# alibaba/easydist

Measured on AMD Instinct MI355X. Metric: gpt2_train_samples_per_sec, higher is better.
Workload: dtype bf16; 1 GPU; model=gpt2-small, global_batch=64, seq_len=1024, parallelism=auto(dp1)

## Files before the change

### easydist_amd/ops/csrc/attn_kernels.hip

```cpp
#include "common.h"
#include "attn_block_map.h"
#include <torch/extension.h>
#include <ATen/cuda/CUDAContext.h>
#include <climits>

using f32x4 = __attribute__((ext_vector_type(4))) float;
using bf16x8v = __attribute__((ext_vector_type(8))) __bf16;

#define QB 64
#define KB 64

DEVINL int lsw(int e) { return e ^ (((e >> 7) & 15) << 3); }


DEVINL void swp_pack(const f32x4* sacc, int nj, unsigned pk[][2]) {
  for (int j = 0; j < nj; ++j)
    #pragma unroll
    for (int t2 = 0; t2 < 2; ++t2)
      asm("v_cvt_pk_bf16_f32 %0, %1, %2"
          : "=v"(pk[j][t2])
          : "v"(sacc[j][2 * t2]), "v"(sacc[j][2 * t2 + 1]));
}

DEVINL bf16x8v swp_butterfly(const unsigned pk[][2], int ks, int fg) {
  unsigned o0 = pk[2 * ks][0], o1 = pk[2 * ks][1];
  unsigned p0 = pk[2 * ks + 1][0], p1 = pk[2 * ks + 1][1];
  const bool g_odd = (fg & 1), g_hi = (fg >= 2);
  unsigned r16a = __shfl_xor((int)(g_odd ? o0 : p0), 16, WAVE);
  unsigned r16b = __shfl_xor((int)(g_odd ? o1 : p1), 16, WAVE);
  unsigned r32a = __shfl_xor((int)(g_hi ? o0 : p0), 32, WAVE);
  unsigned r32b = __shfl_xor((int)(g_hi ? o1 : p1), 32, WAVE);
  unsigned r48a = __shfl_xor((int)(fg == 2 ? o0 : p0), 48, WAVE);
  unsigned r48b = __shfl_xor((int)(fg == 2 ? o1 : p1), 48, WAVE);
  union { unsigned u[4]; bf16x8v v; } cv;
  if (fg == 0) {
    cv.u[0] = o0;  cv.u[1] = o1;  cv.u[2] = r16a; cv.u[3] = r16b;
  } else if (fg == 1) {
    cv.u[0] = r48a; cv.u[1] = r48b; cv.u[2] = r32a; cv.u[3] = r32b;
  } else if (fg == 2) {
    cv.u[0] = r32a; cv.u[1] = r32b; cv.u[2] = r48a; cv.u[3] = r48b;
  } else {
    cv.u[0] = r16a; cv.u[1] = r16b; cv.u[2] = p0;  cv.u[3] = p1;
  }
  return cv.v;
}

template <int D>
__global__ void
__launch_bounds__(512, (D == 64 ? 4 : 1))
flash_fwd_kernel(const bf16* __restrict__ Q, const bf16* __restrict__ K,
                 const bf16* __restrict__ V, bf16* __restrict__ O,
                 float* __restrict__ LSE, int B, int H, int S, bool causal,
                 float scale,
                 long qsb, long qsh, long qss, long ksb, long ksh, long kss,
                 long vsb, long vsh, long vss, int map_mode) {
  constexpr int QBLK = 2 * QB;
  const AttnBlock wgm = attn_block_map(blockIdx.x, (S + QBLK - 1) / QBLK,
                                       B * H, causal, map_mode);
  const int qb0 = wgm.blk * QBLK;
  const int bh = wgm.bh;
  const int b_ = bh / H, h_ = bh % H;
  const bf16* q = Q + b_ * qsb + h_ * qsh;
  const bf16* k = K + b_ * ksb + h_ * ksh;
  const bf16* v = V + b_ * vsb + h_ * vsh;
  bf16* o = O + (long)bh * S * D;
  float* lse = LSE + (long)bh * S;

  const int lane = threadIdx.x % WAVE;
  const int wave = threadIdx.x / WAVE;

  extern __shared__ __attribute__((aligned(16))) char smem[];
  constexpr int TILE_K = KB * D;
  constexpr int TILE_VT = KB * D;
  bf16* smem_b = reinterpret_cast<bf16*>(smem);
  constexpr int NTHR = 8 * WAVE;

  const int fr = lane & 15;
  const int fg = lane >> 4;

  const int qr0 = qb0 + wave * 16;
  const int qrow = qr0 + fr;

  const float qscale = scale * 1.44269504088896340736f;
  bf16x8v qf[D / 32];
  #pragma unroll
  for (int ks = 0; ks < D / 32; ++ks) {
    if (qrow < S) {
      bf16x8v raw = *reinterpret_cast<const bf16x8v*>(
          &q[(long)qrow * qss + ks * 32 + fg * 8]);
      #pragma unroll
      for (int u = 0; u < 8; ++u)
        qf[ks][u] = (__bf16)(bf2f((bf16)raw[u]) * qscale);
    } else {
      #pragma unroll
      for (int u = 0; u < 8; ++u) qf[ks][u] = (__bf16)0.f;
    }
  }

  float m_run = -1e30f, l_run = 0.f;
  f32x4 o_acc[D / 16];
  #pragma unroll
  for (int j = 0; j < D / 16; ++j) o_acc[j] = {0.f, 0.f, 0.f, 0.f};

  const int kv_end = causal ? min(S, qb0 + QBLK) : S;
  const int n_tiles = (kv_end + KB - 1) / KB;
  constexpr int PF = TILE_K / (NTHR * 8);
  bf16x8 kreg[PF], vreg[PF];

  auto load_tile = [&](int t) {
    #pragma unroll
    for (int pi = 0; pi < PF; ++pi) {
      const int e = threadIdx.x * 8 + pi * (NTHR * 8);
      const int row = t * KB + e / D, col = e % D;
      kreg[pi] = *reinterpret_cast<const bf16x8*>(&k[(long)row * kss + col]);
      vreg[pi] = *reinterpret_cast<const bf16x8*>(&v[(long)row * vss + col]);
    }
  };
  auto store_tile = [&](int t) {
    bf16* kb = smem_b + (t & 1) * (TILE_K + TILE_VT);
    bf16* vb = kb + TILE_K;
    #pragma unroll
    for (int pi = 0; pi < PF; ++pi) {
      const int e = threadIdx.x * 8 + pi * (NTHR * 8);
      *reinterpret_cast<bf16x8*>(&kb[lsw(e)]) = kreg[pi];
      const int row = e / D, col = e % D;
      #pragma unroll
      for (int i = 0; i < 8; ++i)
        vb[lsw((col + i) * KB + row)] = vreg[pi].v[i];
    }
  };

  load_tile(0);
  store_tile(0);
  __syncthreads();

  for (int t = 0; t < n_tiles; ++t) {
    const int kv0 = t * KB;
    const bf16* k_lds = smem_b + (t & 1) * (TILE_K + TILE_VT);
    const bf16* vt_lds = k_lds + TILE_K;
    if (t + 1 < n_tiles)
      load_tile(t + 1);

    const bool wave_active = !(causal && kv0 > qr0 + 15);
    if (wave_active) {
      f32x4 s_acc[KB / 16];
      __builtin_amdgcn_s_setprio(1);
      #pragma unroll
      for (int j = 0; j < KB / 16; ++j) {
        s_acc[j] = {0.f, 0.f, 0.f, 0.f};
        #pragma unroll
        for (int ks = 0; ks < D / 32; ++ks) {
          bf16x8v kf = *reinterpret_cast<const bf16x8v*>(
              &k_lds[lsw((j * 16 + fr) * D + ks * 32 + fg * 8)]);
          s_acc[j] = __builtin_amdgcn_mfma_f32_16x16x32_bf16(
              kf, qf[ks], s_acc[j], 0, 0, 0);
        }
      }
      __builtin_amdgcn_s_setprio(0);
      const bool need_mask = (causal && kv0 + KB - 1 > qrow)
                             || (kv0 + KB > S);
      float mx = -1e30f;
      if (need_mask) {
        #pragma unroll
        for (int j = 0; j < KB / 16; ++j)
          #pragma unroll
          for (int r = 0; r < 4; ++r) {
            int kcol = kv0 + j * 16 + 4 * fg + r;
            float sv = s_acc[j][r];
            if ((causal && kcol > qrow) || kcol >= S) sv = -1e30f;
            s_acc[j][r] = sv;
            mx = fmaxf(mx, sv);
          }
      } else {
        #pragma unroll
        for (int j = 0; j < KB / 16; ++j)
          #pragma unroll
          for (int r = 0; r < 4; ++r) mx = fmaxf(mx, s_acc[j][r]);
      }
      mx = fmaxf(mx, __shfl_xor(mx, 16, WAVE));
      mx = fmaxf(mx, __shfl_xor(mx, 32, WAVE));
      float m_new = fmaxf(m_run, mx);
      float psum = 0.f;
      #pragma unroll
      for (int j = 0; j < KB / 16; ++j)
        #pragma unroll
        for (int r = 0; r < 4; ++r) {
          float pp = __builtin_amdgcn_exp2f(s_acc[j][r] - m_new);
          s_acc[j][r] = pp;
          psum += pp;
        }
      psum += __shfl_xor(psum, 16, WAVE);
      psum += __shfl_xor(psum, 32, WAVE);
      float alpha = __builtin_amdgcn_exp2f(m_run - m_new);
      l_run = l_run * alpha + psum;
      m_run = m_new;
      #pragma unroll
      for (int r = 0; r < 4; ++r) {
        float ar = __shfl(alpha, 4 * fg + r, WAVE);
        #pragma unroll
        for (int j = 0; j < D / 16; ++j) o_acc[j][r] *= ar;
      }
      unsigned pk[KB / 16][2];
      swp_pack(s_acc, KB / 16, pk);
      __builtin_amdgcn_s_setprio(1);
      #pragma unroll
      for (int ks = 0; ks < KB / 32; ++ks) {
        bf16x8v pv = swp_butterfly(pk, ks, fg);
        #pragma unroll
        for (int j = 0; j < D / 16; ++j) {
          bf16x8v vf = *reinterpret_cast<const bf16x8v*>(
              &vt_lds[lsw((j * 16 + fr) * KB + ks * 32 + fg * 8)]);
          o_acc[j] = __builtin_amdgcn_mfma_f32_16x16x32_bf16(
              pv, vf, o_acc[j], 0, 0, 0);
        }
      }
      __builtin_amdgcn_s_setprio(0);
    }

    if (t + 1 < n_tiles)
      store_tile(t + 1);
    __syncthreads();
  }

  float invl = 1.f / l_run;
  #pragma unroll
  for (int r = 0; r < 4; ++r) {
    int orow = qr0 + 4 * fg + r;
    if (orow >= S) continue;
    float ir = __shfl(invl, 4 * fg + r, WAVE);
    #pragma unroll
    for (int j = 0; j < D / 16; ++j)
      o[(long)orow * D + j * 16 + fr] = f2bf(o_acc[j][r] * ir);
  }
  if (fg == 0 && qrow < S)
    lse[qrow] = 0.69314718055994530942f * (m_run + __log2f(l_run));
}

static inline at::Tensor ed_attn_arg(const at::Tensor& t) {
  return t.stride(3) == 1 ? t : t.contiguous();
}

static inline int ed_attn_map_mode() {
  const char* e = getenv("EASYDIST_ATTN_MAP");
  return (e && atoi(e) == 0) ? ATTN_MAP_LEGACY : ATTN_MAP_BALANCED;
}

static inline dim3 ed_attn_grid(long nblk, long nbh, const char* who) {
  TORCH_CHECK(nblk * nbh <= (long)INT_MAX, who,
              ": workgroup count ", nblk * nbh, " does not fit in an int");
  return dim3((unsigned)(nblk * nbh));
}

std::tuple<at::Tensor, at::Tensor> flash_attn_fwd(const at::Tensor& q_,
                                                  const at::Tensor& k_,
                                                  const at::Tensor& v_,
                                                  bool causal) {
  auto q = ed_attn_arg(q_), k = ed_attn_arg(k_), v = ed_attn_arg(v_);
  TORCH_CHECK(q.dtype() == at::kBFloat16 && q.dim() == 4);
  TORCH_CHECK(q.sizes() == k.sizes() && q.sizes() == v.sizes(),
              "flash_attn_fwd: q/k/v shapes must match");
  const int B = q.size(0), H = q.size(1), S = q.size(2), D = q.size(3);
  TORCH_CHECK(D == 64 || D == 128, "flash_attn_fwd: D in {64,128}");
  TORCH_CHECK(S % QB == 0, "flash_attn_fwd: S multiple of 64");
  auto out = at::empty({B, H, S, D}, q.options());
  auto lse = at::empty({B, H, S}, q.options().dtype(at::kFloat));
  auto stream = at::cuda::getCurrentCUDAStream();
  dim3 grid = ed_attn_grid((S + 2 * QB - 1) / (2 * QB), (long)B * H,
                           "flash_attn_fwd"), block(512);
  const int map_mode = ed_attn_map_mode();
  size_t lds = (2 * ((size_t)KB * D + (size_t)KB * D) + 8 * 16 * KB) * 2;
  float scale = 1.f / sqrtf((float)D);
  auto kern = (D == 64) ? flash_fwd_kernel<64> : flash_fwd_kernel<128>;
  hipLaunchKernelGGL(kern, grid, block, lds, stream,
      (const bf16*)q.data_ptr(), (const bf16*)k.data_ptr(),
      (const bf16*)v.data_ptr(), (bf16*)out.data_ptr(),
      lse.data_ptr<float>(), B, H, S, causal, scale,
      q.stride(0), q.stride(1), q.stride(2),
      k.stride(0), k.stride(1), k.stride(2),
      v.stride(0), v.stride(1), v.stride(2), map_mode);
  return {out, lse};
}


template <int D>
__global__ void __launch_bounds__(512)
flash_bwd_dq_kernel(const bf16* __restrict__ dO, const bf16* __restrict__ Q,
                    const bf16* __restrict__ K, const bf16* __restrict__ V,
                    const float* __restrict__ LSE,
                    const float* __restrict__ DELTA, bf16* __restrict__ DQ,
                    int B, int H, int S, bool causal, float scale,
                    long dsb, long dsh, long dss, long qsb, long qsh,
                    long qss, long ksb, long ksh, long kss, long vsb,
                    long vsh, long vss, long osb, long osh, long oss,
                    int map_mode) {
  const AttnBlock wgm = attn_block_map(blockIdx.x, S / (2 * QB), B * H,
                                       causal, map_mode);
  const int qb0 = wgm.blk * (2 * QB);
  const int bh = wgm.bh;
  const int b_ = bh / H, h_ = bh % H;
  const bf16* dO_ = dO + b_ * dsb + h_ * dsh;
  const bf16* q = Q + b_ * qsb + h_ * qsh;
  const bf16* k = K + b_ * ksb + h_ * ksh;
  const bf16* v = V + b_ * vsb + h_ * vsh;
  bf16* dq = DQ + b_ * osb + h_ * osh;
  const float* lse = LSE + (long)bh * S;
  const float* delta = DELTA + (long)bh * S;

  const int lane = threadIdx.x % WAVE;
  const int wave = threadIdx.x / WAVE;
  const int qr0 = qb0 + wave * 16;
  const int fr = lane & 15;
  const int fg = lane >> 4;

  extern __shared__ __attribute__((aligned(16))) char smem[];
  constexpr int DQBUF = 3 * KB * D;
  bf16* k_lds = reinterpret_cast<bf16*>(smem);
  bf16* v_lds = k_lds + KB * D;
  bf16* kt_lds = v_lds + KB * D;

  bf16x8v qf[D / 32], dof[D / 32];
  #pragma unroll
  for (int ks = 0; ks < D / 32; ++ks) {
    qf[ks] = *reinterpret_cast<const bf16x8v*>(
        &q[(long)(qr0 + fr) * qss + ks * 32 + fg * 8]);
    dof[ks] = *reinterpret_cast<const bf16x8v*>(
        &dO_[(long)(qr0 + fr) * dss + ks * 32 + fg * 8]);
  }
  const int qrow = qr0 + fr;
  const float lse_r = lse[qrow];
  const float dlt_r = delta[qrow];

  f32x4 dq_acc[D / 16];
  #pragma unroll
  for (int j = 0; j < D / 16; ++j) dq_acc[j] = {0.f, 0.f, 0.f, 0.f};

  const int kv_end = causal ? min(S, qb0 + 2 * QB) : S;
  constexpr int NV = KB * D / (512 * 8);
  bf16x8 kreg[NV], vreg[NV];
  auto kv_load = [&](int t0) {
    #pragma unroll
    for (int pi = 0; pi < NV; ++pi) {
      const int e = threadIdx.x * 8 + pi * 4096;
      const long row = t0 + e / D;
      const int col = e % D;
      kreg[pi] = *reinterpret_cast<const bf16x8*>(&k[row * kss + col]);
      vreg[pi] = *reinterpret_cast<const bf16x8*>(&v[row * vss + col]);
    }
  };
  auto kv_store = [&](int buf) {
    #pragma unroll
    for (int pi = 0; pi < NV; ++pi) {
      const int e = threadIdx.x * 8 + pi * 4096;
      *reinterpret_cast<bf16x8*>(&k_lds[buf * DQBUF + lsw(e)]) = kreg[pi];
      *reinterpret_cast<bf16x8*>(&v_lds[buf * DQBUF + lsw(e)]) = vreg[pi];
      const int row = e / D, col = e % D;
      #pragma unroll
      for (int i = 0; i < 8; ++i)
        kt_lds[buf * DQBUF + lsw((col + i) * KB + row)] = kreg[pi].v[i];
    }
  };
  kv_load(0);
  kv_store(0);
  __syncthreads();
  const int n_kt = (kv_end + KB - 1) / KB;
  for (int tt = 0; tt < n_kt; ++tt) {
    const int kv0 = tt * KB;
    const int bofs = (tt & 1) * DQBUF;
    if (tt + 1 < n_kt) kv_load(kv0 + KB);
    if (causal && kv0 > qr0 + 15) {
      if (tt + 1 < n_kt) kv_store((tt + 1) & 1);
      __syncthreads();
      continue;
    }

    f32x4 s_acc[KB / 16], dp_acc[KB / 16];
    #pragma unroll
    for (int j = 0; j < KB / 16; ++j) {
      s_acc[j] = {0.f, 0.f, 0.f, 0.f};
      dp_acc[j] = {0.f, 0.f, 0.f, 0.f};
      #pragma unroll
      for (int ks = 0; ks < D / 32; ++ks) {
        bf16x8v kf = *reinterpret_cast<const bf16x8v*>(
            &k_lds[bofs + lsw((j * 16 + fr) * D + ks * 32 + fg * 8)]);
        bf16x8v vf = *reinterpret_cast<const bf16x8v*>(
            &v_lds[bofs + lsw((j * 16 + fr) * D + ks * 32 + fg * 8)]);
        s_acc[j] = __builtin_amdgcn_mfma_f32_16x16x32_bf16(
            kf, qf[ks], s_acc[j], 0, 0, 0);
        dp_acc[j] = __builtin_amdgcn_mfma_f32_16x16x32_bf16(
            vf, dof[ks], dp_acc[j], 0, 0, 0);
      }
    }
    const bool need_mask = (causal && kv0 + KB - 1 > qrow)
                           || (kv0 + KB > S);
    #pragma unroll
    for (int j = 0; j < KB / 16; ++j)
      #pragma unroll
      for (int r = 0; r < 4; ++r) {
        float p = 0.f;
        int kcol = kv0 + j * 16 + 4 * fg + r;
        if (!need_mask || (!(causal && kcol > qrow) && kcol < S))
          p = __expf(s_acc[j][r] * scale - lse_r);
        s_acc[j][r] = p * (dp_acc[j][r] - dlt_r) * scale;
      }
    bf16x8v dsf[KB / 32];
    unsigned pk[KB / 16][2];
    swp_pack(s_acc, KB / 16, pk);
    #pragma unroll
    for (int ks = 0; ks < KB / 32; ++ks)
      dsf[ks] = swp_butterfly(pk, ks, fg);
    #pragma unroll
    for (int j = 0; j < D / 16; ++j) {
      #pragma unroll
      for (int ks = 0; ks < KB / 32; ++ks) {
        bf16x8v kcol = *reinterpret_cast<const bf16x8v*>(
            &kt_lds[bofs + lsw((j * 16 + fr) * KB + ks * 32 + fg * 8)]);
        dq_acc[j] = __builtin_amdgcn_mfma_f32_16x16x32_bf16(dsf[ks], kcol,
                                                            dq_acc[j], 0, 0,
                                                            0);
      }
    }
    if (tt + 1 < n_kt) kv_store((tt + 1) & 1);
    __syncthreads();
  }
  #pragma unroll
  for (int r = 0; r < 4; ++r) {
    int orow = qr0 + 4 * fg + r;
    if (orow >= S) continue;
    #pragma unroll
    for (int j = 0; j < D / 16; ++j)
      dq[(long)orow * oss + j * 16 + fr] = f2bf(dq_acc[j][r]);
  }
}

template <int D, int SW = 0>
__global__ void __launch_bounds__(512)
flash_bwd_dkv_kernel(const bf16* __restrict__ dO, const bf16* __restrict__ Q,
                     const bf16* __restrict__ K, const bf16* __restrict__ V,
                     const float* __restrict__ LSE,
                     const float* __restrict__ DELTA, bf16* __restrict__ DK,
                     bf16* __restrict__ DV, int B, int H, int S, bool causal,
                     float scale,
                     long dsb, long dsh, long dss, long qsb, long qsh,
                     long qss, long ksb, long ksh, long kss, long vsb,
                     long vsh, long vss, long osb, long osh, long oss,
                     int map_mode) {
  const AttnBlock wgm = attn_block_map(blockIdx.x, S / (2 * KB), B * H,
                                       false, map_mode);
  const int kb0 = wgm.blk * (2 * KB);
  const int bh = wgm.bh;
  const int b_ = bh / H, h_ = bh % H;
  const bf16* dO_ = dO + b_ * dsb + h_ * dsh;
  const bf16* q = Q + b_ * qsb + h_ * qsh;
  const bf16* k = K + b_ * ksb + h_ * ksh;
  const bf16* v = V + b_ * vsb + h_ * vsh;
  bf16* dk = DK + b_ * osb + h_ * osh;
  bf16* dv = DV + b_ * osb + h_ * osh;
  const float* lse = LSE + (long)bh * S;
  const float* delta = DELTA + (long)bh * S;

  const int lane = threadIdx.x % WAVE;
  const int wave = threadIdx.x / WAVE;
  const int kr0 = kb0 + wave * 16;
  const int fr = lane & 15;
  const int fg = lane >> 4;

  extern __shared__ __attribute__((aligned(16))) char smem[];
  constexpr int KVBUF = 4 * QB * D;
  bf16* q_lds = reinterpret_cast<bf16*>(smem);
  bf16* do_lds = q_lds + QB * D;
  bf16* qt_lds = do_lds + QB * D;
  bf16* dot_lds = qt_lds + QB * D;
  bf16* s_lds = reinterpret_cast<bf16*>(smem) + 2 * KVBUF + wave * 16 * QB;

  bf16x8v kf[D / 32], vf[D / 32];
  #pragma unroll
  for (int ks = 0; ks < D / 32; ++ks) {
    kf[ks] = *reinterpret_cast<const bf16x8v*>(
        &k[(long)(kr0 + fr) * kss + ks * 32 + fg * 8]);
    vf[ks] = *reinterpret_cast<const bf16x8v*>(
        &v[(long)(kr0 + fr) * vss + ks * 32 + fg * 8]);
  }

  f32x4 dk_acc[D / 16], dv_acc[D / 16];
  #pragma unroll
  for (int j = 0; j < D / 16; ++j) {
    dk_acc[j] = {0.f, 0.f, 0.f, 0.f};
    dv_acc[j] = {0.f, 0.f, 0.f, 0.f};
  }

  const int q_start = causal ? kb0 : 0;
  constexpr int NV = QB * D / (512 * 8);
  bf16x8 qreg[NV], dreg[NV];
  auto q_load = [&](int t0) {
    #pragma unroll
    for (int pi = 0; pi < NV; ++pi) {
      const int e = threadIdx.x * 8 + pi * 4096;
      const long row = t0 + e / D;
      const int col = e % D;
      qreg[pi] = *reinterpret_cast<const bf16x8*>(&q[row * qss + col]);
      dreg[pi] = *reinterpret_cast<const bf16x8*>(&dO_[row * dss + col]);
    }
  };
  auto q_store = [&](int buf) {
    #pragma unroll
    for (int pi = 0; pi < NV; ++pi) {
      const int e = threadIdx.x * 8 + pi * 4096;
      *reinterpret_cast<bf16x8*>(&q_lds[buf * KVBUF + lsw(e)]) = qreg[pi];
      *reinterpret_cast<bf16x8*>(&do_lds[buf * KVBUF + lsw(e)]) = dreg[pi];
      const int row = e / D, col = e % D;
      #pragma unroll
      for (int i = 0; i < 8; ++i) {
        qt_lds[buf * KVBUF + lsw((col + i) * QB + row)] = qreg[pi].v[i];
        dot_lds[buf * KVBUF + lsw((col + i) * QB + row)] = dreg[pi].v[i];
      }
    }
  };
  q_load(q_start);
  q_store(0);
  __syncthreads();
  const int n_qt = (S - q_start + QB - 1) / QB;
  for (int tt = 0; tt < n_qt; ++tt) {
    const int q0 = q_start + tt * QB;
    const int bofs = (tt & 1) * KVBUF;
    if (tt + 1 < n_qt) q_load(q0 + QB);
    if (causal && q0 + QB - 1 < kr0) {
      if (tt + 1 < n_qt) q_store((tt + 1) & 1);
      __syncthreads();
      continue;
    }

    f32x4 st_acc[QB / 16], dpt_acc[QB / 16];
    #pragma unroll
    for (int j = 0; j < QB / 16; ++j) {
      st_acc[j] = {0.f, 0.f, 0.f, 0.f};
      dpt_acc[j] = {0.f, 0.f, 0.f, 0.f};
      #pragma unroll
      for (int ks = 0; ks < D / 32; ++ks) {
        bf16x8v qfb = *reinterpret_cast<const bf16x8v*>(
            &q_lds[bofs + lsw((j * 16 + fr) * D + ks * 32 + fg * 8)]);
        bf16x8v dob = *reinterpret_cast<const bf16x8v*>(
            &do_lds[bofs + lsw((j * 16 + fr) * D + ks * 32 + fg * 8)]);
        if (SW) {
          st_acc[j] = __builtin_amdgcn_mfma_f32_16x16x32_bf16(
              qfb, kf[ks], st_acc[j], 0, 0, 0);
          dpt_acc[j] = __builtin_amdgcn_mfma_f32_16x16x32_bf16(
              dob, vf[ks], dpt_acc[j], 0, 0, 0);
        } else {
          st_acc[j] = __builtin_amdgcn_mfma_f32_16x16x32_bf16(
              kf[ks], qfb, st_acc[j], 0, 0, 0);
          dpt_acc[j] = __builtin_amdgcn_mfma_f32_16x16x32_bf16(
              vf[ks], dob, dpt_acc[j], 0, 0, 0);
        }
      }
    }
    bf16x8v ptf[QB / 32];
    const bool need_mask = (causal && kr0 + 15 > q0) || (q0 + QB > S);
    if (SW) {
      const int krow = kr0 + fr;
      #pragma unroll
      for (int j = 0; j < QB / 16; ++j) {
        f32x4 l4 = *reinterpret_cast<const f32x4*>(
            &lse[q0 + j * 16 + 4 * fg]);
        #pragma unroll
        for (int r = 0; r < 4; ++r) {
          int qcol = q0 + j * 16 + 4 * fg + r;
          float p = 0.f;
          if (!need_mask || (!(causal && krow > qcol) && qcol < S))
            p = __expf(st_acc[j][r] * scale - l4[r]);
          st_acc[j][r] = p;
        }
      }
      unsigned pk[QB / 16][2];
      swp_pack(st_acc, QB / 16, pk);
      #pragma unroll
      for (int ks = 0; ks < QB / 32; ++ks)
        ptf[ks] = swp_butterfly(pk, ks, fg);
    } else {
    if (need_mask) {
      #pragma unroll
      for (int j = 0; j < QB / 16; ++j) {
        int qcol = q0 + j * 16 + fr;
        float l = lse[qcol];
        #pragma unroll
        for (int r = 0; r < 4; ++r) {
          int krow = kr0 + 4 * fg + r;
          float p = 0.f;
          if (!(causal && krow > qcol) && qcol < S)
            p = __expf(st_acc[j][r] * scale - l);
          st_acc[j][r] = p;
          s_lds[lsw((4 * fg + r) * QB + j * 16 + fr)] = f2bf(p);
        }
      }
    } else {
      #pragma unroll
      for (int j = 0; j < QB / 16; ++j) {
        float l = lse[q0 + j * 16 + fr];
        #pragma unroll
        for (int r = 0; r < 4; ++r) {
          float p = __expf(st_acc[j][r] * scale - l);
          st_acc[j][r] = p;
          s_lds[lsw((4 * fg + r) * QB + j * 16 + fr)] = f2bf(p);
        }
      }
    }
    lds_fence();
    #pragma unroll
    for (int ks = 0; ks < QB / 32; ++ks)
      ptf[ks] = *reinterpret_cast<const bf16x8v*>(
          &s_lds[lsw(fr * QB + ks * 32 + fg * 8)]);
    }
    #pragma unroll
    for (int j = 0; j < D / 16; ++j) {
      #pragma unroll
      for (int ks = 0; ks < QB / 32; ++ks) {
        bf16x8v docol = *reinterpret_cast<const bf16x8v*>(
            &dot_lds[bofs + lsw((j * 16 + fr) * QB + ks * 32 + fg * 8)]);
        dv_acc[j] = __builtin_amdgcn_mfma_f32_16x16x32_bf16(ptf[ks], docol,
                                                            dv_acc[j], 0, 0,
                                                            0);
      }
    }
    bf16x8v dstf[QB / 32];
    if (SW) {
      #pragma unroll
      for (int j = 0; j < QB / 16; ++j) {
        f32x4 d4 = *reinterpret_cast<const f32x4*>(
            &delta[q0 + j * 16 + 4 * fg]);
        #pragma unroll
        for (int r = 0; r < 4; ++r) {
          float ds = st_acc[j][r] * (dpt_acc[j][r] - d4[r]) * scale;
          st_acc[j][r] = ds;
        }
      }
      unsigned pk2[QB / 16][2];
      swp_pack(st_acc, QB / 16, pk2);
      #pragma unroll
      for (int ks = 0; ks < QB / 32; ++ks)
        dstf[ks] = swp_butterfly(pk2, ks, fg);
    } else {
    lds_fence();
    #pragma unroll
    for (int j = 0; j < QB / 16; ++j) {
      int qcol = q0 + j * 16 + fr;
      float dlt = delta[qcol];
      #pragma unroll
      for (int r = 0; r < 4; ++r) {
        float ds = st_acc[j][r] * (dpt_acc[j][r] - dlt) * scale;
        s_lds[lsw((4 * fg + r) * QB + j * 16 + fr)] = f2bf(ds);
      }
    }
    lds_fence();
    #pragma unroll
    for (int ks = 0; ks < QB / 32; ++ks)
      dstf[ks] = *reinterpret_cast<const bf16x8v*>(
          &s_lds[lsw(fr * QB + ks * 32 + fg * 8)]);
    }
    #pragma unroll
    for (int j = 0; j < D / 16; ++j) {
      #pragma unroll
      for (int ks = 0; ks < QB / 32; ++ks) {
        bf16x8v qcolf = *reinterpret_cast<const bf16x8v*>(
            &qt_lds[bofs + lsw((j * 16 + fr) * QB + ks * 32 + fg * 8)]);
        dk_acc[j] = __builtin_amdgcn_mfma_f32_16x16x32_bf16(dstf[ks], qcolf,
                                                            dk_acc[j], 0, 0,
                                                            0);
      }
    }
    if (tt + 1 < n_qt) q_store((tt + 1) & 1);
    __syncthreads();
  }
  #pragma unroll
  for (int r = 0; r < 4; ++r) {
    int krow = kr0 + 4 * fg + r;
    if (krow >= S) continue;
    #pragma unroll
    for (int j = 0; j < D / 16; ++j) {
      dk[(long)krow * oss + j * 16 + fr] = f2bf(dk_acc[j][r]);
      dv[(long)krow * oss + j * 16 + fr] = f2bf(dv_acc[j][r]);
    }
  }
}

template <int D>
__global__ void __launch_bounds__(256)
attn_delta_kernel(const bf16* __restrict__ dO, const bf16* __restrict__ O,
                  float* __restrict__ delta, long rows, int H, int S,
                  long dsb, long dsh, long dss) {
  constexpr int LPR = D / 8;
  const int lane = threadIdx.x % WAVE;
  const int wave = threadIdx.x / WAVE;
  constexpr int RPW = WAVE / LPR;
  long row = (long)blockIdx.x * (4 * RPW) + wave * RPW + lane / LPR;
  if (row >= rows) return;
  const int c0 = (lane % LPR) * 8;
  const long b_ = row / ((long)H * S), hs = row % ((long)H * S);
  const long h_ = hs / S, s_ = hs % S;
  const bf16x8 d8 = *reinterpret_cast<const bf16x8*>(
      &dO[b_ * dsb + h_ * dsh + s_ * dss + c0]);
  const bf16x8 o8 = *reinterpret_cast<const bf16x8*>(&O[row * D + c0]);
  float acc = 0.f;
  #pragma unroll
  for (int i = 0; i < 8; ++i) acc += bf2f(d8.v[i]) * bf2f(o8.v[i]);
  #pragma unroll
  for (int off = LPR / 2; off > 0; off >>= 1)
    acc += __shfl_down(acc, off, WAVE);
  if (lane % LPR == 0) delta[row] = acc;
}

static void
flash_attn_bwd_launch(const at::Tensor& grad_, const at::Tensor& q_,
                      const at::Tensor& k_, const at::Tensor& v_,
                      const at::Tensor& out, const at::Tensor& lse,
                      bool causal, bf16* dq_p, bf16* dk_p, bf16* dv_p,
                      long osb, long osh, long oss) {
  auto grad = ed_attn_arg(grad_);
  auto q = ed_attn_arg(q_), k = ed_attn_arg(k_), v = ed_attn_arg(v_);
  TORCH_CHECK(q.dtype() == at::kBFloat16 && q.dim() == 4);
  TORCH_CHECK(q.sizes() == k.sizes() && q.sizes() == v.sizes());
  TORCH_CHECK(out.is_contiguous(), "flash_attn_bwd: out must be contiguous");
  const int B = q.size(0), H = q.size(1), S = q.size(2), D = q.size(3);
  TORCH_CHECK(D == 64 || D == 128, "flash_attn_bwd: D in {64,128}");
  TORCH_CHECK(S % (2 * QB) == 0, "flash_attn_bwd: S multiple of 128");
  auto delta = at::empty({B, H, S}, q.options().dtype(at::kFloat));
  {
    long rows = (long)B * H * S;
    int rpw = (D == 64) ? 8 : 4;
    long nblk = (rows + 4 * rpw - 1) / (4 * rpw);
    auto stream0 = at::cuda::getCurrentCUDAStream();
    auto dkern = (D == 64) ? attn_delta_kernel<64> : attn_delta_kernel<128>;
    hipLaunchKernelGGL(dkern, dim3(nblk), dim3(256), 0,
        stream0, (const bf16*)grad.data_ptr(), (const bf16*)out.data_ptr(),
        delta.data_ptr<float>(), rows, H, S,
        grad.stride(0), grad.stride(1), grad.stride(2));
  }
  auto stream = at::cuda::getCurrentCUDAStream();
  dim3 grid = ed_attn_grid(S / (2 * QB), (long)B * H, "flash_attn_bwd"),
       block(512);
  const int map_mode = ed_attn_map_mode();
  size_t lds = (2 * (3 * (size_t)KB * D) + 8 * 16 * KB) * 2;
  size_t lds_kv = (2 * (4 * (size_t)QB * D) + 8 * 16 * QB) * 2;
  float scale = 1.f / sqrtf((float)D);
  auto qkern = (D == 64) ? flash_bwd_dq_kernel<64> : flash_bwd_dq_kernel<128>;
  static int swkv = []() {
    const char* e = getenv("EASYDIST_DKV_SWAP");
    return e ? atoi(e) : 0;
  }();
  auto kkern = (D == 64)
      ? (swkv ? flash_bwd_dkv_kernel<64, 1> : flash_bwd_dkv_kernel<64>)
      : (swkv ? flash_bwd_dkv_kernel<128, 1> : flash_bwd_dkv_kernel<128>);
  hipLaunchKernelGGL(qkern, grid, block, lds, stream,
      (const bf16*)grad.data_ptr(), (const bf16*)q.data_ptr(),
      (const bf16*)k.data_ptr(), (const bf16*)v.data_ptr(),
      lse.data_ptr<float>(), delta.data_ptr<float>(),
      dq_p, B, H, S, causal, scale,
      grad.stride(0), grad.stride(1), grad.stride(2),
      q.stride(0), q.stride(1), q.stride(2),
      k.stride(0), k.stride(1), k.stride(2),
      v.stride(0), v.stride(1), v.stride(2), osb, osh, oss, map_mode);
  hipLaunchKernelGGL(kkern, grid, block, lds_kv, stream,
      (const bf16*)grad.data_ptr(), (const bf16*)q.data_ptr(),
      (const bf16*)k.data_ptr(), (const bf16*)v.data_ptr(),
      lse.data_ptr<float>(), delta.data_ptr<float>(),
      dk_p, dv_p, B, H, S, causal, scale,
      grad.stride(0), grad.stride(1), grad.stride(2),
      q.stride(0), q.stride(1), q.stride(2),
      k.stride(0), k.stride(1), k.stride(2),
      v.stride(0), v.stride(1), v.stride(2), osb, osh, oss, map_mode);
}

std::tuple<at::Tensor, at::Tensor, at::Tensor>
flash_attn_bwd(const at::Tensor& grad_, const at::Tensor& q_,
               const at::Tensor& k_, const at::Tensor& v_,
               const at::Tensor& out, const at::Tensor& lse, bool causal) {
  const int B = q_.size(0), H = q_.size(1), S = q_.size(2), D = q_.size(3);
  auto opts = q_.options();
  auto dq = at::empty({B, H, S, D}, opts);
  auto dk = at::empty({B, H, S, D}, opts);
  auto dv = at::empty({B, H, S, D}, opts);
  flash_attn_bwd_launch(grad_, q_, k_, v_, out, lse, causal,
                        (bf16*)dq.data_ptr(), (bf16*)dk.data_ptr(),
                        (bf16*)dv.data_ptr(),
                        (long)H * S * D, (long)S * D, D);
  return {dq, dk, dv};
}

at::Tensor
flash_attn_bwd_pack(const at::Tensor& grad_, const at::Tensor& q_,
                    const at::Tensor& k_, const at::Tensor& v_,
                    const at::Tensor& out, const at::Tensor& lse,
                    bool causal) {
  const long B = q_.size(0), H = q_.size(1), S = q_.size(2), D = q_.size(3);
  auto dqkv = at::empty({B, S, 3 * H * D}, q_.options());
  bf16* base = (bf16*)dqkv.data_ptr();
  flash_attn_bwd_launch(grad_, q_, k_, v_, out, lse, causal,
                        base, base + H * D, base + 2 * H * D,
                        S * 3 * H * D, D, 3 * H * D);
  return dqkv;
}
```

Baseline: 756.7 samples/sec.

## Use ds_read_tr16 transposed LDS reads instead of storing transposed tile copies

Result: faster. 773.6 samples/sec (median of 6 runs) (+2.2%).

```diff
diff --git a/easydist_amd/ops/csrc/attn_kernels.hip b/easydist_amd/ops/csrc/attn_kernels.hip
--- a/easydist_amd/ops/csrc/attn_kernels.hip
+++ b/easydist_amd/ops/csrc/attn_kernels.hip
@@ -3,6 +3,7 @@
 #include <torch/extension.h>
 #include <ATen/cuda/CUDAContext.h>
 #include <climits>
+#include <type_traits>
 
 using f32x4 = __attribute__((ext_vector_type(4))) float;
 using bf16x8v = __attribute__((ext_vector_type(8))) __bf16;
@@ -11,6 +12,52 @@
 #define KB 64
 
 DEVINL int lsw(int e) { return e ^ (((e >> 7) & 15) << 3); }
+
+template <int D>
+DEVINL int tsw(int e) {
+  const int r = e / D;
+  const int g = (((r & 1) << 3) | (((r >> 3) & 1) << 2) | (((r >> 1) & 1) << 1))
+                & (D / 8 - 1);
+  return e ^ (g << 3);
+}
+template <int D, bool TR>
+DEVINL int isw(int e) {
+  if constexpr (TR) return tsw<D>(e);
+  else return lsw(e);
+}
+
+using v4s = __attribute__((ext_vector_type(4))) short;
+using v8s = __attribute__((ext_vector_type(8))) short;
+struct TrLane { int off, x; };
+template <int D, bool TR>
+DEVINL TrLane tr_lane(int fr, int fg) {
+  if constexpr (!TR) return {0, 0};
+  const int e = (fg * 8 + (fr >> 2)) * D + (fr & 3) * 4;
+  return {e, tsw<D>(e) ^ e};
+}
+template <int D>
+DEVINL bf16x8v tr_frag(const bf16* img, TrLane tl, int r0, int c0) {
+  const bf16* a = img + ((c0 ^ tl.x) + tl.off) + r0 * D;
+  v4s lo = __builtin_amdgcn_ds_read_tr16_b64_v4i16(
+      (__attribute__((address_space(3))) v4s*)a);
+  v4s hi = __builtin_amdgcn_ds_read_tr16_b64_v4i16(
+      (__attribute__((address_space(3))) v4s*)(a + 4 * D));
+  v8s out = __builtin_shufflevector(lo, hi, 0, 1, 2, 3, 4, 5, 6, 7);
+  return __builtin_bit_cast(bf16x8v, out);
+}
+
+template <bool TR>
+using stage_t = std::conditional_t<TR, bf16x8v, bf16x8>;
+
+template <int D, bool TR> constexpr int fwd_lds_elems() {
+  return 2 * (2 * KB * D) + (TR ? 0 : 8 * 16 * KB);
+}
+template <int D, bool TR> constexpr int dq_lds_elems() {
+  return 2 * ((TR ? 2 : 3) * KB * D) + (TR ? 0 : 8 * 16 * KB);
+}
+template <int D, bool TR> constexpr int dkv_lds_elems() {
+  return 2 * ((TR ? 2 : 4) * QB * D) + 8 * 16 * QB;
+}
 
 
 DEVINL void swp_pack(const f32x4* sacc, int nj, unsigned pk[][2]) {
@@ -45,7 +92,7 @@
   return cv.v;
 }
 
-template <int D>
+template <int D, bool TR>
 __global__ void
 __launch_bounds__(512, (D == 64 ? 4 : 1))
 flash_fwd_kernel(const bf16* __restrict__ Q, const bf16* __restrict__ K,
@@ -72,11 +119,13 @@
   extern __shared__ __attribute__((aligned(16))) char smem[];
   constexpr int TILE_K = KB * D;
   constexpr int TILE_VT = KB * D;
+  static_assert(2 * (TILE_K + TILE_VT) <= fwd_lds_elems<D, TR>());
   bf16* smem_b = reinterpret_cast<bf16*>(smem);
   constexpr int NTHR = 8 * WAVE;
 
   const int fr = lane & 15;
   const int fg = lane >> 4;
+  const TrLane trl = tr_lane<D, TR>(fr, fg);
 
   const int qr0 = qb0 + wave * 16;
   const int qrow = qr0 + fr;
@@ -105,15 +154,17 @@
   const int kv_end = causal ? min(S, qb0 + QBLK) : S;
   const int n_tiles = (kv_end + KB - 1) / KB;
   constexpr int PF = TILE_K / (NTHR * 8);
-  bf16x8 kreg[PF], vreg[PF];
+  stage_t<TR> kreg[PF], vreg[PF];
 
   auto load_tile = [&](int t) {
     #pragma unroll
     for (int pi = 0; pi < PF; ++pi) {
       const int e = threadIdx.x * 8 + pi * (NTHR * 8);
       const int row = t * KB + e / D, col = e % D;
-      kreg[pi] = *reinterpret_cast<const bf16x8*>(&k[(long)row * kss + col]);
-      vreg[pi] = *reinterpret_cast<const bf16x8*>(&v[(long)row * vss + col]);
+      kreg[pi] = *reinterpret_cast<const stage_t<TR>*>(
+          &k[(long)row * kss + col]);
+      vreg[pi] = *reinterpret_cast<const stage_t<TR>*>(
+          &v[(long)row * vss + col]);
     }
   };
   auto store_tile = [&](int t) {
@@ -122,11 +173,15 @@
     #pragma unroll
     for (int pi = 0; pi < PF; ++pi) {
       const int e = threadIdx.x * 8 + pi * (NTHR * 8);
-      *reinterpret_cast<bf16x8*>(&kb[lsw(e)]) = kreg[pi];
-      const int row = e / D, col = e % D;
-      #pragma unroll
-      for (int i = 0; i < 8; ++i)
-        vb[lsw((col + i) * KB + row)] = vreg[pi].v[i];
+      *reinterpret_cast<stage_t<TR>*>(&kb[isw<D, TR>(e)]) = kreg[pi];
+      if constexpr (TR) {
+        *reinterpret_cast<bf16x8v*>(&vb[tsw<D>(e)]) = vreg[pi];
+      } else {
+        const int row = e / D, col = e % D;
+        #pragma unroll
+        for (int i = 0; i < 8; ++i)
+          vb[lsw((col + i) * KB + row)] = vreg[pi].v[i];
+      }
     }
   };
 
@@ -151,7 +206,7 @@
         #pragma unroll
         for (int ks = 0; ks < D / 32; ++ks) {
           bf16x8v kf = *reinterpret_cast<const bf16x8v*>(
-              &k_lds[lsw((j * 16 + fr) * D + ks * 32 + fg * 8)]);
+              &k_lds[isw<D, TR>((j * 16 + fr) * D + ks * 32 + fg * 8)]);
           s_acc[j] = __builtin_amdgcn_mfma_f32_16x16x32_bf16(
               kf, qf[ks], s_acc[j], 0, 0, 0);
         }
@@ -208,8 +263,12 @@
         bf16x8v pv = swp_butterfly(pk, ks, fg);
         #pragma unroll
         for (int j = 0; j < D / 16; ++j) {
-          bf16x8v vf = *reinterpret_cast<const bf16x8v*>(
-              &vt_lds[lsw((j * 16 + fr) * KB + ks * 32 + fg * 8)]);
+          bf16x8v vf;
+          if constexpr (TR)
+            vf = tr_frag<D>(vt_lds, trl, ks * 32, j * 16);
+          else
+            vf = *reinterpret_cast<const bf16x8v*>(
+                &vt_lds[lsw((j * 16 + fr) * KB + ks * 32 + fg * 8)]);
           o_acc[j] = __builtin_amdgcn_mfma_f32_16x16x32_bf16(
               pv, vf, o_acc[j], 0, 0, 0);
         }
@@ -243,6 +302,14 @@
 static inline int ed_attn_map_mode() {
   const char* e = getenv("EASYDIST_ATTN_MAP");
   return (e && atoi(e) == 0) ? ATTN_MAP_LEGACY : ATTN_MAP_BALANCED;
+}
+
+#define ATTN_TR_FWD 1
+#define ATTN_TR_DQ 1
+#define ATTN_TR_DKV(D) ((D) == 128)
+static inline bool ed_attn_tr(bool dflt) {
+  const char* e = getenv("EASYDIST_ATTN_TR");
+  return e ? atoi(e) != 0 : dflt;
 }
 
 static inline dim3 ed_attn_grid(long nblk, long nbh, const char* who) {
@@ -268,9 +335,15 @@
   dim3 grid = ed_attn_grid((S + 2 * QB - 1) / (2 * QB), (long)B * H,
                            "flash_attn_fwd"), block(512);
   const int map_mode = ed_attn_map_mode();
-  size_t lds = (2 * ((size_t)KB * D + (size_t)KB * D) + 8 * 16 * KB) * 2;
+  const bool tr = ed_attn_tr(ATTN_TR_FWD);
+  size_t lds = sizeof(bf16) *
+      (D == 64 ? (tr ? fwd_lds_elems<64, true>() : fwd_lds_elems<64, false>())
+               : (tr ? fwd_lds_elems<128, true>()
+                     : fwd_lds_elems<128, false>()));
   float scale = 1.f / sqrtf((float)D);
-  auto kern = (D == 64) ? flash_fwd_kernel<64> : flash_fwd_kernel<128>;
+  auto kern = (D == 64)
+      ? (tr ? flash_fwd_kernel<64, true> : flash_fwd_kernel<64, false>)
+      : (tr ? flash_fwd_kernel<128, true> : flash_fwd_kernel<128, false>);
   hipLaunchKernelGGL(kern, grid, block, lds, stream,
       (const bf16*)q.data_ptr(), (const bf16*)k.data_ptr(),
       (const bf16*)v.data_ptr(), (bf16*)out.data_ptr(),
@@ -282,7 +355,7 @@
 }
 
 
-template <int D>
+template <int D, bool TR>
 __global__ void __launch_bounds__(512)
 flash_bwd_dq_kernel(const bf16* __restrict__ dO, const bf16* __restrict__ Q,
                     const bf16* __restrict__ K, const bf16* __restrict__ V,
@@ -311,9 +384,11 @@
   const int qr0 = qb0 + wave * 16;
   const int fr = lane & 15;
   const int fg = lane >> 4;
+  const TrLane trl = tr_lane<D, TR>(fr, fg);
 
   extern __shared__ __attribute__((aligned(16))) char smem[];
-  constexpr int DQBUF = 3 * KB * D;
+  constexpr int DQBUF = (TR ? 2 : 3) * KB * D;
+  static_assert(2 * DQBUF <= dq_lds_elems<D, TR>());
   bf16* k_lds = reinterpret_cast<bf16*>(smem);
   bf16* v_lds = k_lds + KB * D;
   bf16* kt_lds = v_lds + KB * D;
@@ -336,27 +411,31 @@
 
   const int kv_end = causal ? min(S, qb0 + 2 * QB) : S;
   constexpr int NV = KB * D / (512 * 8);
-  bf16x8 kreg[NV], vreg[NV];
+  stage_t<TR> kreg[NV], vreg[NV];
   auto kv_load = [&](int t0) {
     #pragma unroll
     for (int pi = 0; pi < NV; ++pi) {
       const int e = threadIdx.x * 8 + pi * 4096;
       const long row = t0 + e / D;
       const int col = e % D;
-      kreg[pi] = *reinterpret_cast<const bf16x8*>(&k[row * kss + col]);
-      vreg[pi] = *reinterpret_cast<const bf16x8*>(&v[row * vss + col]);
+      kreg[pi] = *reinterpret_cast<const stage_t<TR>*>(&k[row * kss + col]);
+      vreg[pi] = *reinterpret_cast<const stage_t<TR>*>(&v[row * vss + col]);
     }
   };
   auto kv_store = [&](int buf) {
     #pragma unroll
     for (int pi = 0; pi < NV; ++pi) {
       const int e = threadIdx.x * 8 + pi * 4096;
-      *reinterpret_cast<bf16x8*>(&k_lds[buf * DQBUF + lsw(e)]) = kreg[pi];
-      *reinterpret_cast<bf16x8*>(&v_lds[buf * DQBUF + lsw(e)]) = vreg[pi];
-      const int row = e / D, col = e % D;
-      #pragma unroll
-      for (int i = 0; i < 8; ++i)
-        kt_lds[buf * DQBUF + lsw((col + i) * KB + row)] = kreg[pi].v[i];
+      *reinterpret_cast<stage_t<TR>*>(
+          &k_lds[buf * DQBUF + isw<D, TR>(e)]) = kreg[pi];
+      *reinterpret_cast<stage_t<TR>*>(
+          &v_lds[buf * DQBUF + isw<D, TR>(e)]) = vreg[pi];
+      if constexpr (!TR) {
+        const int row = e / D, col = e % D;
+        #pragma unroll
+        for (int i = 0; i < 8; ++i)
+          kt_lds[buf * DQBUF + lsw((col + i) * KB + row)] = kreg[pi].v[i];
+      }
     }
   };
   kv_load(0);
@@ -381,9 +460,9 @@
       #pragma unroll
       for (int ks = 0; ks < D / 32; ++ks) {
         bf16x8v kf = *reinterpret_cast<const bf16x8v*>(
-            &k_lds[bofs + lsw((j * 16 + fr) * D + ks * 32 + fg * 8)]);
+            &k_lds[bofs + isw<D, TR>((j * 16 + fr) * D + ks * 32 + fg * 8)]);
         bf16x8v vf = *reinterpret_cast<const bf16x8v*>(
-            &v_lds[bofs + lsw((j * 16 + fr) * D + ks * 32 + fg * 8)]);
+            &v_lds[bofs + isw<D, TR>((j * 16 + fr) * D + ks * 32 + fg * 8)]);
         s_acc[j] = __builtin_amdgcn_mfma_f32_16x16x32_bf16(
             kf, qf[ks], s_acc[j], 0, 0, 0);
         dp_acc[j] = __builtin_amdgcn_mfma_f32_16x16x32_bf16(
@@ -412,8 +491,12 @@
     for (int j = 0; j < D / 16; ++j) {
       #pragma unroll
       for (int ks = 0; ks < KB / 32; ++ks) {
-        bf16x8v kcol = *reinterpret_cast<const bf16x8v*>(
-            &kt_lds[bofs + lsw((j * 16 + fr) * KB + ks * 32 + fg * 8)]);
+        bf16x8v kcol;
+        if constexpr (TR)
+          kcol = tr_frag<D>(k_lds + bofs, trl, ks * 32, j * 16);
+        else
+          kcol = *reinterpret_cast<const bf16x8v*>(
+              &kt_lds[bofs + lsw((j * 16 + fr) * KB + ks * 32 + fg * 8)]);
         dq_acc[j] = __builtin_amdgcn_mfma_f32_16x16x32_bf16(dsf[ks], kcol,
                                                             dq_acc[j], 0, 0,
                                                             0);
@@ -432,7 +515,7 @@
   }
 }
 
-template <int D, int SW = 0>
+template <int D, int SW, bool TR>
 __global__ void __launch_bounds__(512)
 flash_bwd_dkv_kernel(const bf16* __restrict__ dO, const bf16* __restrict__ Q,
                      const bf16* __restrict__ K, const bf16* __restrict__ V,
@@ -463,9 +546,11 @@
   const int kr0 = kb0 + wave * 16;
   const int fr = lane & 15;
   const int fg = lane >> 4;
+  const TrLane trl = tr_lane<D, TR>(fr, fg);
 
   extern __shared__ __attribute__((aligned(16))) char smem[];
-  constexpr int KVBUF = 4 * QB * D;
+  constexpr int KVBUF = (TR ? 2 : 4) * QB * D;
+  static_assert(2 * KVBUF + 8 * 16 * QB == dkv_lds_elems<D, TR>());
   bf16* q_lds = reinterpret_cast<bf16*>(smem);
   bf16* do_lds = q_lds + QB * D;
   bf16* qt_lds = do_lds + QB * D;
@@ -490,28 +575,33 @@
 
   const int q_start = causal ? kb0 : 0;
   constexpr int NV = QB * D / (512 * 8);
-  bf16x8 qreg[NV], dreg[NV];
+  stage_t<TR> qreg[NV], dreg[NV];
   auto q_load = [&](int t0) {
     #pragma unroll
     for (int pi = 0; pi < NV; ++pi) {
       const int e = threadIdx.x * 8 + pi * 4096;
       const long row = t0 + e / D;
       const int col = e % D;
-      qreg[pi] = *reinterpret_cast<const bf16x8*>(&q[row * qss + col]);
-      dreg[pi] = *reinterpret_cast<const bf16x8*>(&dO_[row * dss + col]);
+      qreg[pi] = *reinterpret_cast<const stage_t<TR>*>(&q[row * qss + col]);
+      dreg[pi] = *reinterpret_cast<const stage_t<TR>*>(
+          &dO_[row * dss + col]);
     }
   };
   auto q_store = [&](int buf) {
     #pragma unroll
     for (int pi = 0; pi < NV; ++pi) {
       const int e = threadIdx.x * 8 + pi * 4096;
-      *reinterpret_cast<bf16x8*>(&q_lds[buf * KVBUF + lsw(e)]) = qreg[pi];
-      *reinterpret_cast<bf16x8*>(&do_lds[buf * KVBUF + lsw(e)]) = dreg[pi];
-      const int row = e / D, col = e % D;
-      #pragma unroll
-      for (int i = 0; i < 8; ++i) {
-        qt_lds[buf * KVBUF + lsw((col + i) * QB + row)] = qreg[pi].v[i];
-        dot_lds[buf * KVBUF + lsw((col + i) * QB + row)] = dreg[pi].v[i];
+      *reinterpret_cast<stage_t<TR>*>(
+          &q_lds[buf * KVBUF + isw<D, TR>(e)]) = qreg[pi];
+      *reinterpret_cast<stage_t<TR>*>(
+          &do_lds[buf * KVBUF + isw<D, TR>(e)]) = dreg[pi];
+      if constexpr (!TR) {
+        const int row = e / D, col = e % D;
+        #pragma unroll
+        for (int i = 0; i < 8; ++i) {
+          qt_lds[buf * KVBUF + lsw((col + i) * QB + row)] = qreg[pi].v[i];
+          dot_lds[buf * KVBUF + lsw((col + i) * QB + row)] = dreg[pi].v[i];
+        }
       }
     }
   };
@@ -537,9 +627,9 @@
       #pragma unroll
       for (int ks = 0; ks < D / 32; ++ks) {
         bf16x8v qfb = *reinterpret_cast<const bf16x8v*>(
-            &q_lds[bofs + lsw((j * 16 + fr) * D + ks * 32 + fg * 8)]);
+            &q_lds[bofs + isw<D, TR>((j * 16 + fr) * D + ks * 32 + fg * 8)]);
         bf16x8v dob = *reinterpret_cast<const bf16x8v*>(
-            &do_lds[bofs + lsw((j * 16 + fr) * D + ks * 32 + fg * 8)]);
+            &do_lds[bofs + isw<D, TR>((j * 16 + fr) * D + ks * 32 + fg * 8)]);
         if (SW) {
           st_acc[j] = __builtin_amdgcn_mfma_f32_16x16x32_bf16(
               qfb, kf[ks], st_acc[j], 0, 0, 0);
@@ -613,8 +703,12 @@
     for (int j = 0; j < D / 16; ++j) {
       #pragma unroll
       for (int ks = 0; ks < QB / 32; ++ks) {
-        bf16x8v docol = *reinterpret_cast<const bf16x8v*>(
-            &dot_lds[bofs + lsw((j * 16 + fr) * QB + ks * 32 + fg * 8)]);
+        bf16x8v docol;
+        if constexpr (TR)
+          docol = tr_frag<D>(do_lds + bofs, trl, ks * 32, j * 16);
+        else
+          docol = *reinterpret_cast<const bf16x8v*>(
+              &dot_lds[bofs + lsw((j * 16 + fr) * QB + ks * 32 + fg * 8)]);
         dv_acc[j] = __builtin_amdgcn_mfma_f32_16x16x32_bf16(ptf[ks], docol,
                                                             dv_acc[j], 0, 0,
                                                             0);
@@ -659,8 +753,12 @@
     for (int j = 0; j < D / 16; ++j) {
       #pragma unroll
       for (int ks = 0; ks < QB / 32; ++ks) {
-        bf16x8v qcolf = *reinterpret_cast<const bf16x8v*>(
-            &qt_lds[bofs + lsw((j * 16 + fr) * QB + ks * 32 + fg * 8)]);
+        bf16x8v qcolf;
+        if constexpr (TR)
+          qcolf = tr_frag<D>(q_lds + bofs, trl, ks * 32, j * 16);
+        else
+          qcolf = *reinterpret_cast<const bf16x8v*>(
+              &qt_lds[bofs + lsw((j * 16 + fr) * QB + ks * 32 + fg * 8)]);
         dk_acc[j] = __builtin_amdgcn_mfma_f32_16x16x32_bf16(dstf[ks], qcolf,
                                                             dk_acc[j], 0, 0,
                                                             0);
@@ -737,17 +835,34 @@
   dim3 grid = ed_attn_grid(S / (2 * QB), (long)B * H, "flash_attn_bwd"),
        block(512);
   const int map_mode = ed_attn_map_mode();
-  size_t lds = (2 * (3 * (size_t)KB * D) + 8 * 16 * KB) * 2;
-  size_t lds_kv = (2 * (4 * (size_t)QB * D) + 8 * 16 * QB) * 2;
+  const bool tr_q = ed_attn_tr(ATTN_TR_DQ), tr_kv = ed_attn_tr(ATTN_TR_DKV(D));
+  size_t lds = sizeof(bf16) *
+      (D == 64 ? (tr_q ? dq_lds_elems<64, true>() : dq_lds_elems<64, false>())
+               : (tr_q ? dq_lds_elems<128, true>()
+                       : dq_lds_elems<128, false>()));
+  size_t lds_kv = sizeof(bf16) *
+      (D == 64 ? (tr_kv ? dkv_lds_elems<64, true>()
+                        : dkv_lds_elems<64, false>())
+               : (tr_kv ? dkv_lds_elems<128, true>()
+                        : dkv_lds_elems<128, false>()));
   float scale = 1.f / sqrtf((float)D);
-  auto qkern = (D == 64) ? flash_bwd_dq_kernel<64> : flash_bwd_dq_kernel<128>;
+  auto qkern = (D == 64)
+      ? (tr_q ? flash_bwd_dq_kernel<64, true> : flash_bwd_dq_kernel<64, false>)
+      : (tr_q ? flash_bwd_dq_kernel<128, true>
+              : flash_bwd_dq_kernel<128, false>);
   static int swkv = []() {
     const char* e = getenv("EASYDIST_DKV_SWAP");
     return e ? atoi(e) : 0;
   }();
   auto kkern = (D == 64)
-      ? (swkv ? flash_bwd_dkv_kernel<64, 1> : flash_bwd_dkv_kernel<64>)
-      : (swkv ? flash_bwd_dkv_kernel<128, 1> : flash_bwd_dkv_kernel<128>);
+      ? (swkv ? (tr_kv ? flash_bwd_dkv_kernel<64, 1, true>
+                       : flash_bwd_dkv_kernel<64, 1, false>)
+              : (tr_kv ? flash_bwd_dkv_kernel<64, 0, true>
+                       : flash_bwd_dkv_kernel<64, 0, false>))
+      : (swkv ? (tr_kv ? flash_bwd_dkv_kernel<128, 1, true>
+                       : flash_bwd_dkv_kernel<128, 1, false>)
+              : (tr_kv ? flash_bwd_dkv_kernel<128, 0, true>
+                       : flash_bwd_dkv_kernel<128, 0, false>));
   hipLaunchKernelGGL(qkern, grid, block, lds, stream,
       (const bf16*)grad.data_ptr(), (const bf16*)q.data_ptr(),
       (const bf16*)k.data_ptr(), (const bf16*)v.data_ptr(),
```
